# c0rv4x/zkevm-prover

Measured on AMD Instinct MI355X. Metric: batch-proof STARK sec (2^23 trace) + Goldilocks NTT Gelem/s at 1/2/4/8 GPU, lower is better.
Workload: dtype u64 (Goldilocks) + F_p^3

## Files before the change

### zkevm-prover_amd/csrc/ntt.hip

```cpp
#include <stdlib.h>
#include <string.h>

#include <algorithm>
#include <utility>
#include <vector>

#include "gl_device.hpp"
#include "gl_rb.hpp"
#include "zkgpu_internal.hpp"

namespace zk {

__global__ void k_fill_powers(uint64_t *out, uint64_t base, uint64_t step, uint64_t scale, uint64_t count)
{
    uint64_t i = (uint64_t)blockIdx.x * blockDim.x + threadIdx.x;
    if (i >= count) return;
    uint64_t b = gl_pow(base, step);
    out[i] = gl_canon(gl_mul(scale, gl_pow(b, i)));
}

__device__ __forceinline__ uint32_t bitrev_u32(uint32_t x, uint32_t bits)
{
    return bits == 0 ? 0 : (__builtin_bitreverse32(x) >> (32 - bits));
}

__device__ __forceinline__ uint64_t tw_big(const uint64_t *lo, const uint64_t *hi, uint64_t e)
{
    return gl_mul(lo[e & (TW_LEVEL_SIZE - 1)], hi[e >> TW_LEVEL_BITS]);
}

struct PassArgs {
    const uint64_t *src;
    uint64_t src_ld;
    uint64_t src_valid;
    uint32_t half_zero;
    uint64_t *dst;
    uint64_t dst_ld;
    const uint64_t *tw_lo;
    const uint64_t *tw_hi;
    const uint64_t *post_lo;
    const uint64_t *post_hi;
    uint64_t post_step;
    uint64_t post_scale;
    uint32_t post_bits;
    uint32_t logn;
    uint32_t logm;
    uint32_t last;
    uint32_t npass;
    uint32_t rbits[NTT_MAX_PASSES];
    const uint64_t *otw;
    const uint64_t *rt4096;
    uint32_t ncols;
};

constexpr int GROUPS = 16;

#ifndef ZKGPU_NTT_RB
#define ZKGPU_NTT_RB 1
#endif
#ifndef ZKGPU_NTT_RB_SHIFT
#define ZKGPU_NTT_RB_SHIFT 1
#endif
template <bool RB>
__device__ __forceinline__ uint64_t bf_add(uint64_t a, uint64_t b)
{
    if constexpr (RB && ZKGPU_NTT_RB) return gl_add_rb(a, b);
    else return gl_add(a, b);
}
template <bool RB>
__device__ __forceinline__ uint64_t bf_sub(uint64_t a, uint64_t b)
{
    if constexpr (RB && ZKGPU_NTT_RB) return gl_sub_rb(a, b);
    else return gl_sub(a, b);
}

template <int E, bool RB>
__device__ __forceinline__ uint64_t bf_mul2e(uint64_t x)
{
    if constexpr (RB && ZKGPU_NTT_RB && ZKGPU_NTT_RB_SHIFT) return mul2e_rb<E>(x);
    else return mul2e<E>(x);
}

template <bool INV, int H, int I, bool RB>
__device__ __forceinline__ uint64_t dif_odd(uint64_t a, uint64_t c)
{
    constexpr int e = (96 * I) / H;
    if constexpr (e == 0) return bf_sub<RB>(a, c);
    else if constexpr (!INV) return bf_mul2e<e, RB>(bf_sub<RB>(a, c));
    else return bf_mul2e<96 - e, RB>(bf_sub<RB>(c, a));
}

template <int LOG, bool INV, bool RB = false, int H = (1 << LOG) / 2>
__device__ __forceinline__ void dft_regs(uint64_t *v)
{
    if constexpr (H >= 1) {
        constexpr int R = 1 << LOG;
        [&]<int... Bs>(std::integer_sequence<int, Bs...>) {
            (
                [&]<int B>() {
                    [&]<int... Is>(std::integer_sequence<int, Is...>) {
                        (
                            [&]<int I>() {
                                uint64_t a = v[B * 2 * H + I];
                                uint64_t c = v[B * 2 * H + I + H];
                                v[B * 2 * H + I] = bf_add<RB>(a, c);
                                v[B * 2 * H + I + H] = dif_odd<INV, H, I, RB>(a, c);
                            }.template operator()<Is>(),
                            ...);
                    }(std::make_integer_sequence<int, H>{});
                }.template operator()<Bs>(),
                ...);
        }(std::make_integer_sequence<int, R / (2 * H)>{});
        dft_regs<LOG, INV, RB, H / 2>(v);
    }
}

template <int LOG, bool INV, bool RB = false>
__device__ __forceinline__ void dft_regs_half(uint64_t *v)
{
    constexpr int R = 1 << LOG, H = R / 2;
    [&]<int... Is>(std::integer_sequence<int, Is...>) {
        ([&]<int I>() {
            constexpr int e = (96 * I) / H;
            static_assert(!INV, "forward only");
            if constexpr (e == 0) v[I + H] = v[I];
            else v[I + H] = mul2e<e>(v[I]);
        }.template operator()<Is>(), ...);
    }(std::make_integer_sequence<int, H>{});
    dft_regs<LOG, INV, RB, H / 2>(v);
}

__host__ __device__ constexpr int brev_c(int x, int bits)
{
    int r = 0;
    for (int i = 0; i < bits; i++) r |= ((x >> i) & 1) << (bits - 1 - i);
    return r;
}

template <int L1, int L2, bool INV, bool SPLIT>
__global__ void __launch_bounds__(16 * (1 << L2)) k_ntt_pass(PassArgs a)
{
    constexpr int R1 = 1 << L1, R2 = 1 << L2, LOGR = L1 + L2, R = 1 << LOGR;
    constexpr int T = GROUPS * R2;
    __shared__ uint64_t lds[SPLIT ? R * 8 : R * 17];
    uint32_t *lds32 = reinterpret_cast<uint32_t *>(lds);

    __shared__ uint64_t twR[R];
    const uint32_t col = blockIdx.x % a.ncols;
    const uint64_t u = blockIdx.x / a.ncols;
    const uint64_t *src = a.src + (uint64_t)col * a.src_ld;
    uint64_t *dst = a.dst + (uint64_t)col * a.dst_ld;
    const int tid = threadIdx.x;

    static_assert(LOGR <= 12, "radix");
    if (a.rt4096)
        for (int i = tid; i < R; i += T) twR[i] = a.rt4096[i << (12 - LOGR)];
    else
        for (int i = tid; i < R; i += T) twR[i] = tw_big(a.tw_lo, a.tw_hi, (uint64_t)i << (TW_MAX_LOG - LOGR));

    uint64_t v[R2 > R1 ? R2 : R1];
    int g, j2;
    uint64_t base = 0, k1g = 0, rest = 0;
    uint32_t logmp = 0, logS = 0;
    if (!a.last) {
        g = tid & 15;
        j2 = tid >> 4;
        logmp = a.logm - LOGR;
        const uint64_t groups_per_blk = 1ULL << (logmp - 4);
        const uint64_t blk = u >> (logmp - 4);
        const uint64_t j0 = (u & (groups_per_blk - 1)) << 4;
        base = (blk << a.logm) + j0;
#pragma unroll
        for (int j1 = 0; j1 < R1; j1++) {
            uint64_t pos = base + ((uint64_t)(R2 * j1 + j2) << logmp) + g;
            v[j1] = pos < a.src_valid ? src[pos] : 0;
        }
    } else {
        j2 = tid & (R2 - 1);
        g = tid >> L2;
        logS = a.logn - a.rbits[0] - LOGR;
        rest = u & ((1ULL << logS) - 1);
        k1g = u >> logS;
        const uint64_t blk = ((k1g * 16 + g) << logS) + rest;
#pragma unroll
        for (int j1 = 0; j1 < R1; j1++) {
            uint64_t pos = (blk << LOGR) + R2 * j1 + j2;
            v[j1] = pos < a.src_valid ? src[pos] : 0;
        }
    }
    if constexpr (!INV) {
        if (a.half_zero)
            dft_regs_half<L1, INV, true>(v);
        else
            dft_regs<L1, INV, true>(v);
    } else {
        dft_regs<L1, INV, true>(v);
    }
    __syncthreads();
#pragma unroll
    for (int r = 0; r < R1; r++) {
        const int k1 = brev_c(r, L1);
        if (k1) v[r] = gl_mul_rb(v[r], twR[(j2 * k1) & (R - 1)]);
    }
    const bool active = tid < GROUPS * R1;
    const int g2 = tid & 15, k1s = tid >> 4;
    if constexpr (SPLIT) {
        uint32_t lo[R2 > R1 ? R2 : R1];
        const int wb0 = (j2 << 4) + g, wb1 = ((j2 ^ 1) << 4) + g;
        const int fm = (k1s & 1) << 4;
        const int rbe = k1s * R2 * 16 + g2 + fm, rbo = k1s * R2 * 16 + g2 - fm;
#pragma unroll
        for (int r = 0; r < R1; r++) {
            const int k1 = brev_c(r, L1);
            lds32[k1 * R2 * 16 + ((k1 & 1) ? wb1 : wb0)] = (uint32_t)v[r];
        }
        __syncthreads();
        if (active) {
#pragma unroll
            for (int jj = 0; jj < R2; jj++) lo[jj] = lds32[((jj & 1) ? rbo : rbe) + (jj << 4)];
        }
        __syncthreads();
#pragma unroll
        for (int r = 0; r < R1; r++) {
            const int k1 = brev_c(r, L1);
            lds32[k1 * R2 * 16 + ((k1 & 1) ? wb1 : wb0)] = (uint32_t)(v[r] >> 32);
        }
        __syncthreads();
        if (!active) return;
#pragma unroll
        for (int jj = 0; jj < R2; jj++) v[jj] = ((uint64_t)lds32[((jj & 1) ? rbo : rbe) + (jj << 4)] << 32) | lo[jj];
    } else {
#pragma unroll
        for (int r = 0; r < R1; r++) lds[(brev_c(r, L1) * R2 + j2) * 17 + g] = v[r];
        __syncthreads();
        if (!active) return;
#pragma unroll
        for (int jj = 0; jj < R2; jj++) v[jj] = lds[(k1s * R2 + jj) * 17 + g2];
    }
    g = g2;
    const int k1 = k1s;
    dft_regs<L2, INV, true>(v);
    if (!a.last && a.otw) {
        const uint64_t jp = (base & ((1ULL << logmp) - 1)) + g;
#pragma unroll
        for (int k2 = 0; k2 < R2; k2++) {
            const int r = brev_c(k2, L2);
            const uint64_t k = (uint64_t)(k1 + R1 * k2);
            uint64_t x = v[r];
            if (k1 | k2) x = gl_mul_rb(x, a.otw[(k << logmp) + jp]);
            dst[base + (k << logmp) + g] = x;
        }
    } else if (!a.last) {
        const uint32_t tshift = TW_MAX_LOG - a.logm;
        const uint64_t jp = (base & ((1ULL << logmp) - 1)) + g;
        uint64_t t = tw_big(a.tw_lo, a.tw_hi, (jp * k1) << tshift);
        const uint64_t step = tw_big(a.tw_lo, a.tw_hi, (jp * R1) << tshift);
#pragma unroll
        for (int k2 = 0; k2 < R2; k2++) {
            const int r = brev_c(k2, L2);
            uint64_t x = v[r];
            if (k1 | k2) x = gl_mul(x, t);
            dst[base + ((uint64_t)(k1 + R1 * k2) << logmp) + g] = x;
            t = gl_mul(t, step);
        }
    } else {
        uint64_t rrev = 0;
        {
            uint32_t rev_pos[NTT_MAX_PASSES];
            uint32_t acc = 0;
            for (uint32_t i = 1; i + 1 < a.npass; i++) {
                rev_pos[i] = acc;
                acc += a.rbits[i];
            }
            uint64_t rr = rest;
            for (int i = (int)a.npass - 2; i >= 1; i--) {
                uint64_t d = rr & ((1ULL << a.rbits[i]) - 1);
                rr >>= a.rbits[i];
                rrev |= d << rev_pos[i];
            }
        }
        const uint32_t lognr = a.logn - LOGR;
        const uint64_t x0 = (k1g * 16 + g) + (rrev << a.rbits[0]) + ((uint64_t)k1 << lognr);
        const bool scaled = a.post_lo != nullptr || a.post_scale != 1;
        uint64_t f = a.post_scale;
        if (a.post_lo) f = gl_mul(a.post_lo[x0 & ((1ULL << a.post_bits) - 1)], a.post_hi[x0 >> a.post_bits]);
#pragma unroll
        for (int k2 = 0; k2 < R2; k2++) {
            const int r = brev_c(k2, L2);
            uint64_t x = v[r];
            if (scaled) x = gl_mul(x, f);
            dst[x0 + ((uint64_t)(R1 * k2) << lognr)] = gl_canon(x);
            if (a.post_lo) f = gl_mul(f, a.post_step);
        }
    }
}

constexpr int PASS_THREADS = 256;

struct SmallArgs {
    const uint64_t *src;
    uint64_t src_ld;
    uint64_t src_valid;
    uint64_t *dst;
    uint64_t dst_ld;
    const uint64_t *rt_small;
    const uint64_t *post_lo;
    const uint64_t *post_hi;
    uint64_t post_scale;
    uint32_t post_bits;
    uint32_t logn;
};

__global__ void __launch_bounds__(PASS_THREADS) k_ntt_small(SmallArgs a)
{
    __shared__ uint64_t lds[4096];
    const uint32_t col = blockIdx.x;
    const uint64_t *src = a.src + (uint64_t)col * a.src_ld;
    uint64_t *dst = a.dst + (uint64_t)col * a.dst_ld;
    const uint32_t n = 1u << a.logn;
    for (uint32_t i = threadIdx.x; i < n; i += PASS_THREADS) lds[i] = i < a.src_valid ? src[i] : 0;
    for (int lh = (int)a.logn - 1; lh >= 0; lh--) {
        const uint32_t h = 1u << lh;
        __syncthreads();
        for (uint32_t b = threadIdx.x; b < n / 2; b += PASS_THREADS) {
            uint32_t pos = b & (h - 1);
            uint32_t i0 = ((b >> lh) << (lh + 1)) + pos;
            uint32_t i1 = i0 + h;
            uint64_t x = lds[i0], y = lds[i1];
            lds[i0] = gl_add(x, y);
            uint64_t d = gl_sub(x, y);
            lds[i1] = pos == 0 ? d : gl_mul(d, a.rt_small[pos << (11 - lh)]);
        }
    }
    __syncthreads();
    for (uint32_t k = threadIdx.x; k < n; k += PASS_THREADS) {
        uint64_t v = lds[bitrev_u32(k, a.logn)];
        if (a.post_lo)
            v = gl_mul(v, gl_mul(a.post_lo[k & ((1u << a.post_bits) - 1)], a.post_hi[k >> a.post_bits]));
        else if (a.post_scale != 1)
            v = gl_mul(v, a.post_scale);
        dst[k] = gl_canon(v);
    }
}

__global__ void k_rows_to_cols(const uint64_t *__restrict__ in, uint64_t *__restrict__ out, uint64_t nrows,
                               uint64_t ncols, uint64_t ld)
{
    __shared__ uint64_t tile[32][33];
    uint64_t r0 = (uint64_t)blockIdx.x * 32, c0 = (uint64_t)blockIdx.y * 32;
    int tx = threadIdx.x & 31, ty = threadIdx.x >> 5;
    for (int k = ty; k < 32; k += 8) {
        uint64_t r = r0 + k, c = c0 + tx;
        if (r < nrows && c < ncols) tile[k][tx] = in[r * ncols + c];
    }
    __syncthreads();
    for (int k = ty; k < 32; k += 8) {
        uint64_t c = c0 + k, r = r0 + tx;
        if (r < nrows && c < ncols) out[c * ld + r] = tile[tx][k];
    }
}

__global__ void k_cols_to_rows(const uint64_t *__restrict__ in, uint64_t *__restrict__ out, uint64_t nrows,
                               uint64_t ncols, uint64_t ld)
{
    __shared__ uint64_t tile[32][33];
    uint64_t r0 = (uint64_t)blockIdx.x * 32, c0 = (uint64_t)blockIdx.y * 32;
    int tx = threadIdx.x & 31, ty = threadIdx.x >> 5;
    for (int k = ty; k < 32; k += 8) {
        uint64_t c = c0 + k, r = r0 + tx;
        if (r < nrows && c < ncols) tile[k][tx] = in[c * ld + r];
    }
    __syncthreads();
    for (int k = ty; k < 32; k += 8) {
        uint64_t r = r0 + k, c = c0 + tx;
        if (r < nrows && c < ncols) out[r * ncols + c] = tile[tx][k];
    }
}

__global__ void k_otw_table(uint64_t *out, const uint64_t *tw_lo, const uint64_t *tw_hi, uint32_t logm,
                            uint32_t logr)
{
    const uint64_t i = (uint64_t)blockIdx.x * blockDim.x + threadIdx.x;
    if (i >> logm) return;
    const uint32_t logmp = logm - logr;
    const uint64_t k = i >> logmp, jp = i & ((1ULL << logmp) - 1);
    out[i] = gl_canon(tw_big(tw_lo, tw_hi, (jp * k) << (TW_MAX_LOG - logm)));
}

constexpr uint32_t OTW_MAX_LOG = 24;
struct OtwTable {
    int d;
    uint32_t logm, logr;
    uint64_t *ptr;
};
static std::vector<OtwTable> g_otw;

static const uint64_t *otw_table(Ctx &ctx, int d, uint32_t logm, uint32_t logr, hipStream_t s)
{
    if (logm > OTW_MAX_LOG) return nullptr;
    for (const OtwTable &t : g_otw)
        if (t.d == d && t.logm == logm && t.logr == logr) return t.ptr;
    uint64_t *p = nullptr;
    const uint64_t m = 1ULL << logm;
    if (hipMalloc((void **)&p, m * sizeof(uint64_t)) != hipSuccess) {
        (void)hipGetLastError();
        return nullptr;
    }
    hipLaunchKernelGGL(k_otw_table, dim3((uint32_t)((m + 255) / 256)), dim3(256), 0, s, p, ctx.tw_lo[d], ctx.tw_hi[d],
                       logm, logr);
    g_otw.push_back(OtwTable{d, logm, logr, p});
    return p;
}

static const char *PASS_NAMES[2][9] = {
    {"", "", "", "", "k_ntt_pass<4,fwd>", "k_ntt_pass<5,fwd>", "k_ntt_pass<6,fwd>", "k_ntt_pass<7,fwd>",
     "k_ntt_pass<8,fwd>"},
    {"", "", "", "", "k_ntt_pass<4,inv>", "k_ntt_pass<5,inv>", "k_ntt_pass<6,inv>", "k_ntt_pass<7,inv>",
     "k_ntt_pass<8,inv>"}};
static const char *PASS_NAMES_REC[2][9] = {
    {"", "", "", "", "k_ntt_pass<4,fwd,rec>", "k_ntt_pass<5,fwd,rec>", "k_ntt_pass<6,fwd,rec>",
     "k_ntt_pass<7,fwd,rec>", "k_ntt_pass<8,fwd,rec>"},
    {"", "", "", "", "k_ntt_pass<4,inv,rec>", "k_ntt_pass<5,inv,rec>", "k_ntt_pass<6,inv,rec>",
     "k_ntt_pass<7,inv,rec>", "k_ntt_pass<8,inv,rec>"}};

static bool otw_tables_enabled()
{
    const char *e = getenv("ZKGPU_NTT_OTW");
    return !(e && strcmp(e, "0") == 0);
}

static void split_radix(uint32_t logn, uint32_t *npass, uint32_t rbits[NTT_MAX_PASSES])
{
    uint32_t P = (logn + 7) / 8;
    *npass = P;
    uint32_t base = logn / P, extra = logn % P;
    for (uint32_t i = 0; i < P; i++) rbits[i] = base + (i >= P - extra ? 1 : 0);
}

template <int L1, int L2>
static void launch_pass(const PassArgs &a, uint64_t ncols, int inverse, hipStream_t s)
{
    constexpr int LOGR = L1 + L2;
    uint64_t units = (1ULL << (a.logn - LOGR)) / 16;
    dim3 grid((uint32_t)(units * ncols));
    if (inverse)
        hipLaunchKernelGGL((k_ntt_pass<L1, L2, true, true>), grid, dim3(16 << L2), 0, s, a);
    else
        hipLaunchKernelGGL((k_ntt_pass<L1, L2, false, true>), grid, dim3(16 << L2), 0, s, a);
}

static void dispatch_pass(uint32_t logr, const PassArgs &a, uint64_t ncols, int inverse, hipStream_t s)
{
    switch (logr) {
    case 4: launch_pass<2, 2>(a, ncols, inverse, s); break;
    case 5: launch_pass<2, 3>(a, ncols, inverse, s); break;
    case 6: launch_pass<3, 3>(a, ncols, inverse, s); break;
    case 7: launch_pass<3, 4>(a, ncols, inverse, s); break;
    case 8: launch_pass<4, 4>(a, ncols, inverse, s); break;
    default: break;
    }
}

int ntt_columns(Ctx &ctx, uint64_t *dst, uint64_t dst_ld, const uint64_t *src, uint64_t src_ld, uint64_t src_valid,
                uint64_t *tmp, uint64_t tmp_ld, uint32_t logn, uint64_t ncols, int inverse, const uint64_t *post_lo,
                const uint64_t *post_hi, uint32_t post_bits, uint64_t post_base, uint64_t post_scale, hipStream_t s)
{
    if (ncols == 0) return 0;
    if (logn > TW_MAX_LOG) return set_error(ZKGPU_ERR_ARG, "ntt: log2(n) exceeds %u", TW_MAX_LOG);
    const int d = inverse ? 1 : 0;
    if (logn <= 12) {
        SmallArgs sa;
        sa.src = src;
        sa.src_ld = src_ld;
        sa.src_valid = src_valid;
        sa.dst = dst;
        sa.dst_ld = dst_ld;
        sa.rt_small = ctx.rt_small[d];
        sa.post_lo = post_lo;
        sa.post_hi = post_hi;
        sa.post_bits = post_bits;
        sa.post_scale = post_scale;
        sa.logn = logn;
        for (uint64_t c0 = 0; c0 < ncols; c0 += 65535) {
            uint64_t nc = ncols - c0 < 65535 ? ncols - c0 : 65535;
            SmallArgs b = sa;
            b.src = src + c0 * src_ld;
            b.dst = dst + c0 * dst_ld;
            const uint64_t n = 1ULL << logn;
            const uint64_t nread = (src_valid < n ? src_valid : n);
            prof_begin(s);
            hipLaunchKernelGGL(k_ntt_small, dim3((uint32_t)nc), dim3(PASS_THREADS), 0, s, b);
            prof_end("k_ntt_small", 8.0 * (double)(nread + n) * (double)nc, s);
        }
        return check_launch("k_ntt_small");
    }
    PassArgs a;
    a.rt4096 = ctx.rt_small[d];
    a.tw_lo = ctx.tw_lo[d];
    a.tw_hi = ctx.tw_hi[d];
    a.logn = logn;
    split_radix(logn, &a.npass, a.rbits);
    const bool use_otw = otw_tables_enabled();
    uint32_t logm = logn;
    for (uint32_t p = 0; p < a.npass; p++) {
        a.logm = logm;
        a.last = (p == a.npass - 1);
        a.post_lo = a.last ? post_lo : nullptr;
        a.post_hi = a.last ? post_hi : nullptr;
        a.post_bits = post_bits;
        a.post_scale = a.last ? post_scale : 1;
        const uint32_t rb = a.rbits[p];
        a.post_step = h_pow(post_base, (uint64_t)(1u << (rb / 2)) << (logn - rb));
        a.otw = (a.last || !use_otw) ? nullptr : otw_table(ctx, d, logm, rb, s);
        const char *name = (!a.last && !a.otw) ? PASS_NAMES_REC[d][rb] : PASS_NAMES[d][rb];
        a.half_zero = 0;
        if (p == 0) {
            a.src = src;
            a.src_ld = src_ld;
            a.src_valid = src_valid;
            const uint32_t l1 = rb / 2;
            a.half_zero = (!inverse && l1 >= 1 && src_valid == (1ULL << (logn - 1))) ? 1u : 0u;
        } else {
            a.src = tmp;
            a.src_ld = tmp_ld;
            a.src_valid = ~0ULL;
        }
        if (a.last) {
            a.dst = dst;
            a.dst_ld = dst_ld;
        } else {
            a.dst = tmp;
            a.dst_ld = tmp_ld;
        }
        const uint64_t n = 1ULL << logn;
        const uint64_t nread = (a.src_valid < n ? a.src_valid : n);
        const uint64_t units = (1ULL << (logn - rb)) / 16;
        const uint64_t cmax = std::max<uint64_t>(1, std::min<uint64_t>(65535, (1ULL << 32) / (units * 256)));
        for (uint64_t c0 = 0; c0 < ncols; c0 += cmax) {
            uint64_t nc = ncols - c0 < cmax ? ncols - c0 : cmax;
            PassArgs b = a;
            b.src = a.src + c0 * a.src_ld;
            b.dst = a.dst + c0 * a.dst_ld;
            b.ncols = (uint32_t)nc;
            prof_begin(s);
            dispatch_pass(rb, b, nc, inverse, s);
            prof_end(name, 8.0 * (double)(nread + n) * (double)nc, s);
        }
        logm -= rb;
    }
    return check_launch("k_ntt_pass");
}

void rows_to_cols(const uint64_t *in, uint64_t *out, uint64_t nrows, uint64_t ncols, uint64_t ld, hipStream_t s)
{
    if (!nrows || !ncols) return;
    dim3 grid((uint32_t)((nrows + 31) / 32), (uint32_t)((ncols + 31) / 32));
    hipLaunchKernelGGL(k_rows_to_cols, grid, dim3(256), 0, s, in, out, nrows, ncols, ld);
}

void cols_to_rows(const uint64_t *in, uint64_t *out, uint64_t nrows, uint64_t ncols, uint64_t ld, hipStream_t s)
{
    if (!nrows || !ncols) return;
    dim3 grid((uint32_t)((nrows + 31) / 32), (uint32_t)((ncols + 31) / 32));
    hipLaunchKernelGGL(k_cols_to_rows, grid, dim3(256), 0, s, in, out, nrows, ncols, ld);
}

void fill_powers(uint64_t *out, uint64_t base, uint64_t step, uint64_t scale, uint64_t count, hipStream_t s)
{
    uint32_t blocks = (uint32_t)((count + 255) / 256);
    hipLaunchKernelGGL(k_fill_powers, dim3(blocks), dim3(256), 0, s, out, base, step, scale, count);
}


constexpr int LDE_LB = 12;
constexpr uint64_t LDE_RB = 1ULL << LDE_LB;
constexpr int SP_THREADS = 256;

struct StridedArgs {
    const uint64_t *src;
    uint64_t src_ld;
    uint64_t *dst;
    uint64_t dst_ld;
    uint64_t row_stride;
    const uint64_t *tw_r;
    const uint64_t *otw;
    uint32_t canon;
    uint32_t ncols;
    uint32_t units;
};

template <int LA, bool INV>
__global__ void __launch_bounds__(SP_THREADS) k_lde_strided(StridedArgs a)
{
    constexpr int LT = LA - 6, T = 1 << LT, G = SP_THREADS / T, M = 64 / T;
    constexpr int ROW = T * G + (G < 32 ? G : 0);
    __shared__ uint32_t lds[64 * ROW];
    const uint32_t col = blockIdx.x % a.ncols;
    const uint64_t unit = blockIdx.x / a.ncols;
    const uint64_t g0 = unit * G;
    const int tid = threadIdx.x, g = tid % G, t = tid / G;
    const uint64_t rs = a.row_stride;
    const uint64_t *src = a.src + (uint64_t)col * a.src_ld + g0 + g;
    uint64_t v[64];
#pragma unroll
    for (int j1 = 0; j1 < 64; j1++) v[j1] = src[(uint64_t)(t + T * j1) * rs];
    dft_regs<6, INV>(v);
    if constexpr (T > 1) {
#pragma unroll
        for (int r = 1; r < 64; r++) v[r] = gl_mul(v[r], a.tw_r[t * brev_c(r, 6)]);
    }
    const int wb = t * G + g;
#pragma unroll
    for (int r = 0; r < 64; r++) lds[brev_c(r, 6) * ROW + wb] = (uint32_t)v[r];
    __syncthreads();
    uint32_t nl[64];
#pragma unroll
    for (int m = 0; m < M; m++)
#pragma unroll
        for (int j2 = 0; j2 < T; j2++) nl[m * T + j2] = lds[(t + T * m) * ROW + j2 * G + g];
    __syncthreads();
#pragma unroll
    for (int r = 0; r < 64; r++) lds[brev_c(r, 6) * ROW + wb] = (uint32_t)(v[r] >> 32);
    __syncthreads();
#pragma unroll
    for (int m = 0; m < M; m++)
#pragma unroll
        for (int j2 = 0; j2 < T; j2++)
            v[m * T + j2] = ((uint64_t)lds[(t + T * m) * ROW + j2 * G + g] << 32) | nl[m * T + j2];
#pragma unroll
    for (int m = 0; m < M; m++) dft_regs<LT, INV>(v + m * T);
    uint64_t *dst = a.dst + (uint64_t)col * a.dst_ld + g0 + g;
    const uint64_t *otw = a.otw ? a.otw + g0 + g : nullptr;
#pragma unroll
    for (int m = 0; m < M; m++) {
#pragma unroll
        for (int r = 0; r < T; r++) {
            const uint64_t k = (uint64_t)(t + T * m) + 64 * (uint64_t)brev_c(r, LT);
            uint64_t x = v[m * T + r];
            if (otw) x = gl_mul(x, otw[k * LDE_RB]);
            dst[k * rs] = a.canon ? gl_canon(x) : x;
        }
    }
}

struct MidArgs {
    const uint64_t *src;
    uint64_t src_ld;
    uint64_t *dst;
    uint64_t dst_ld;
    const uint64_t *tw16[2];
    const uint64_t *tw256[2];
    const uint64_t *fs;
    const uint64_t *twa[2];
    const uint64_t *otw;
    uint64_t nblk;
    uint32_t ncols;
};

constexpr int MID_LDS = 16 * 272;

#ifndef ZKGPU_LDE_MID_RB
#define ZKGPU_LDE_MID_RB 0
#endif
__device__ __forceinline__ uint64_t mid_mul(uint64_t a, uint64_t b)
{
    if constexpr (ZKGPU_LDE_MID_RB) return gl_mul_rb(a, b);
    else return gl_mul(a, b);
}

template <bool INV, bool TA>
__device__ __forceinline__ void dft4096_block(uint64_t *v, uint64_t *L, int t, const uint64_t *tw16,
                                              const uint64_t *tw256)
{
    dft_regs<4, INV, ZKGPU_LDE_MID_RB>(v);
    if constexpr (TA) {
#pragma unroll
        for (int r = 0; r < 16; r++) v[r] = mid_mul(v[r], tw16[(brev_c(r, 4) << 8) + t]);
    } else {
#pragma unroll
        for (int r = 1; r < 16; r++) v[r] = mid_mul(v[r], tw16[t * brev_c(r, 4)]);
    }
#pragma unroll
    for (int r = 0; r < 16; r++) L[brev_c(r, 4) * 272 + t] = v[r];
    __syncthreads();
    __builtin_amdgcn_sched_barrier(0);
    const int lo = t & 15, hi = t >> 4;
#pragma unroll
    for (int j1 = 0; j1 < 16; j1++) v[j1] = L[hi * 272 + lo + 16 * j1];
    __syncthreads();
    __builtin_amdgcn_sched_barrier(0);
    dft_regs<4, INV, ZKGPU_LDE_MID_RB>(v);
#pragma unroll
    for (int r = 1; r < 16; r++) v[r] = mid_mul(v[r], tw256[lo * brev_c(r, 4)]);
#pragma unroll
    for (int r = 0; r < 16; r++) L[lo * 257 + brev_c(r, 4) * 16 + hi] = v[r];
    __syncthreads();
    __builtin_amdgcn_sched_barrier(0);
#pragma unroll
    for (int j0 = 0; j0 < 16; j0++) v[j0] = L[j0 * 257 + hi * 16 + lo];
    __syncthreads();
    __builtin_amdgcn_sched_barrier(0);
    dft_regs<4, INV, ZKGPU_LDE_MID_RB>(v);
}

__global__ void __launch_bounds__(256) __attribute__((amdgpu_waves_per_eu(2, 2))) k_lde_mid(MidArgs a)
{
    __shared__ uint64_t L[MID_LDS];
    const int t = threadIdx.x;
    const uint64_t blk = blockIdx.x;
    const uint32_t col = (uint32_t)(blk % a.ncols);
    const uint64_t kA = blk / a.ncols;
    const uint64_t *src = a.src + (uint64_t)col * a.src_ld + kA * LDE_RB + t;
    uint64_t v[16], c[16];
#pragma unroll
    for (int j = 0; j < 16; j++) v[j] = src[256 * j];
    dft4096_block<true, false>(v, L, t, a.tw16[1], a.tw256[1]);
    __builtin_amdgcn_sched_barrier(0);
#pragma unroll
    for (int k = 0; k < 16; k++) c[k] = v[brev_c(k, 4)];
    uint64_t *dst = a.dst + (uint64_t)col * a.dst_ld + kA * 2 * LDE_RB + 2 * t;
    const uint64_t *otw = a.otw + kA * LDE_RB + t;
    const uint64_t RA = a.nblk / a.ncols;
    uint64_t z0[16];
    for (int p = 0; p < 2; p++) {
        const uint64_t *S = a.fs + ((uint64_t)p * RA + kA) * 16;
#pragma unroll
        for (int k = 0; k < 16; k++) v[k] = mid_mul(c[k], S[k]);
        dft4096_block<false, true>(v, L, t, a.twa[p], a.tw256[0]);
        __builtin_amdgcn_sched_barrier(0);
        if (p == 0) {
#pragma unroll
            for (int k = 0; k < 16; k++) z0[k] = v[k];
        }
    }
#pragma unroll
    for (int k = 0; k < 16; k++) {
        const uint64_t w = otw[256 * k];
        HIP_vector_type<unsigned long long, 2> pr;
        pr.x = mid_mul(z0[brev_c(k, 4)], w);
        pr.y = mid_mul(v[brev_c(k, 4)], w);
        *reinterpret_cast<HIP_vector_type<unsigned long long, 2> *>(dst + 512 * k) = pr;
    }
}

struct Lde3Tables {
    uint32_t logn = 0;
    uint64_t *pow16[2] = {nullptr, nullptr}, *pow256[2] = {nullptr, nullptr}, *powR[2] = {nullptr, nullptr};
    uint64_t *fs = nullptr, *twa = nullptr;
};

__global__ void k_lde_fs(uint64_t *fs, uint64_t F, uint64_t ninv, uint64_t RA)
{
    const uint64_t i = (uint64_t)blockIdx.x * blockDim.x + threadIdx.x;
    if (i >= RA * 16) return;
    const uint64_t kA = i >> 4, k = i & 15;
    fs[i] = gl_canon(gl_mul(ninv, gl_pow(F, kA + 256 * RA * k)));
}

__global__ void k_lde_twa(uint64_t *twa, uint64_t F, uint64_t w4096, uint64_t RA)
{
    const uint32_t i = blockIdx.x * blockDim.x + threadIdx.x;
    if (i >= 4096) return;
    const uint64_t k2 = i >> 8, t = i & 255;
    twa[i] = gl_canon(gl_mul(gl_pow(F, RA * t), gl_pow(w4096, t * k2)));
}
static Lde3Tables g_lde3;

static int lde3_tables(Ctx &ctx, uint32_t logn, hipStream_t s)
{
    Lde3Tables &T = g_lde3;
    if (T.logn == logn) return 0;
    const uint32_t la = logn - LDE_LB;
    const uint64_t RA = 1ULL << la, n = 1ULL << logn;
    auto alloc = [&](uint64_t **p, uint64_t count) -> int {
        if (*p) (void)hipFree(*p);
        *p = nullptr;
        if (hipMalloc((void **)p, count * 8) != hipSuccess) return set_error(ZKGPU_ERR_OOM, "lde tables");
        return 0;
    };
    int rc;
    for (int d = 0; d < 2; d++) {
        const uint64_t w16 = d ? h_inv(h_w(12)) : h_w(12), w256 = d ? h_inv(h_w(8)) : h_w(8),
                       wR = d ? h_inv(h_w(la)) : h_w(la);
        if ((rc = alloc(&T.pow16[d], 4096)) || (rc = alloc(&T.pow256[d], 256)) || (rc = alloc(&T.powR[d], RA)))
            return rc;
        fill_powers(T.pow16[d], w16, 1, 1, 4096, s);
        fill_powers(T.pow256[d], w256, 1, 1, 256, s);
        fill_powers(T.powR[d], wR, 1, 1, RA, s);
    }
    if ((rc = alloc(&T.fs, 2 * RA * 16)) || (rc = alloc(&T.twa, 2 * 4096))) return rc;
    const uint64_t ninv = h_inv(n);
    for (int p = 0; p < 2; p++) {
        const uint64_t F = p ? h_mul(7, h_w(logn + 1)) : 7;
        hipLaunchKernelGGL(k_lde_fs, dim3((uint32_t)((RA * 16 + 255) / 256)), dim3(256), 0, s, T.fs + p * RA * 16, F,
                           ninv, RA);
        hipLaunchKernelGGL(k_lde_twa, dim3(16), dim3(256), 0, s, T.twa + p * 4096, F, h_w(12), RA);
    }
    if ((rc = check_launch("lde tables"))) return rc;
    T.logn = logn;
    return 0;
}

template <int LA>
static void launch_strided(const StridedArgs &a, uint64_t units, int inverse, hipStream_t s)
{
    const dim3 grid((uint32_t)(units * a.ncols));
    if (inverse) hipLaunchKernelGGL((k_lde_strided<LA, true>), grid, dim3(SP_THREADS), 0, s, a);
    else hipLaunchKernelGGL((k_lde_strided<LA, false>), grid, dim3(SP_THREADS), 0, s, a);
}

static void dispatch_strided(uint32_t la, StridedArgs a, uint64_t groups, int inverse, hipStream_t s)
{
    const uint64_t units = groups / (SP_THREADS >> (la - 6));
    a.units = (uint32_t)units;
    switch (la) {
    case 6: launch_strided<6>(a, units, inverse, s); break;
    case 7: launch_strided<7>(a, units, inverse, s); break;
    case 8: launch_strided<8>(a, units, inverse, s); break;
    case 9: launch_strided<9>(a, units, inverse, s); break;
    case 10: launch_strided<10>(a, units, inverse, s); break;
    case 11: launch_strided<11>(a, units, inverse, s); break;
    case 12: launch_strided<12>(a, units, inverse, s); break;
    default: break;
    }
}

bool lde3_supported(uint32_t logn, uint32_t loge)
{
    const char *e = getenv("ZKGPU_LDE3");
    const bool enabled = e && atoi(e) != 0;
    return enabled && loge == logn + 1 && logn >= LDE_LB + 6 && logn <= LDE_LB + 12;
}

static const char *P1_NAMES[13] = {"", "", "", "", "", "", "k_lde_p1<6>", "k_lde_p1<7>", "k_lde_p1<8>", "k_lde_p1<9>",
                                   "k_lde_p1<10>", "k_lde_p1<11>", "k_lde_p1<12>"};
static const char *P3_NAMES[13] = {"", "", "", "", "", "", "k_lde_p3<6>", "k_lde_p3<7>", "k_lde_p3<8>", "k_lde_p3<9>",
                                   "k_lde_p3<10>", "k_lde_p3<11>", "k_lde_p3<12>"};

int lde3_columns(Ctx &ctx, uint64_t *out, uint64_t ld_out, const uint64_t *in, uint64_t ld_in, uint64_t *t1,
                 uint32_t logn, uint64_t ncols, hipStream_t s)
{
    if (logn < LDE_LB + 6 || logn > LDE_LB + 12) return set_error(ZKGPU_ERR_ARG, "lde3: unsupported size 2^%u", logn);
    if (ncols == 0) return 0;
    int rc;
    if ((rc = lde3_tables(ctx, logn, s))) return rc;
    const uint32_t la = logn - LDE_LB;
    const uint64_t n = 1ULL << logn, RA = 1ULL << la;
    const uint64_t *otw_inv = otw_table(ctx, 1, logn, la, s), *otw_fwd = otw_table(ctx, 0, logn, la, s);
    if (!otw_inv || !otw_fwd) return set_error(ZKGPU_ERR_OOM, "lde3: twiddle tables");
    const uint64_t cmax = std::min<uint64_t>(65535, (1ULL << 31) / (2 * LDE_RB));
    for (uint64_t c0 = 0; c0 < ncols; c0 += cmax) {
        const uint32_t nc = (uint32_t)std::min<uint64_t>(cmax, ncols - c0);
        StridedArgs p1;
        p1.src = in + c0 * ld_in;
        p1.src_ld = ld_in;
        p1.dst = t1;
        p1.dst_ld = n;
        p1.row_stride = LDE_RB;
        p1.tw_r = g_lde3.powR[1];
        p1.otw = otw_inv;
        p1.canon = 0;
        p1.ncols = nc;
        prof_begin(s);
        dispatch_strided(la, p1, LDE_RB, 1, s);
        prof_end(P1_NAMES[la], 16.0 * (double)n * nc, s);
        MidArgs m;
        m.src = t1;
        m.src_ld = n;
        m.dst = out + c0 * ld_out;
        m.dst_ld = ld_out;
        for (int d = 0; d < 2; d++) {
            m.tw16[d] = g_lde3.pow16[d];
            m.tw256[d] = g_lde3.pow256[d];
            m.twa[d] = g_lde3.twa + d * 4096;
        }
        m.fs = g_lde3.fs;
        m.otw = otw_fwd;
        m.nblk = RA * nc;
        m.ncols = nc;
        prof_begin(s);
        hipLaunchKernelGGL(k_lde_mid, dim3((uint32_t)m.nblk), dim3(256), 0, s, m);
        prof_end("k_lde_mid", 24.0 * (double)n * nc, s);
        StridedArgs p3;
        p3.src = out + c0 * ld_out;
        p3.src_ld = ld_out;
        p3.dst = out + c0 * ld_out;
        p3.dst_ld = ld_out;
        p3.row_stride = 2 * LDE_RB;
        p3.tw_r = g_lde3.powR[0];
        p3.otw = nullptr;
        p3.canon = 1;
        p3.ncols = nc;
        prof_begin(s);
        dispatch_strided(la, p3, 2 * LDE_RB, 0, s);
        prof_end(P3_NAMES[la], 32.0 * (double)n * nc, s);
    }
    return check_launch("lde3");
}

}
```

Before: 0.2404.

## Specialize NTT pass kernel by role, input and post mode with scalar-base addressing

Splits the NTT pass kernel into compile-time variants for twiddle-table, recomputed-twiddle and last passes, for full, half-zero and bounds-checked inputs, and for each post-scaling mode, removing runtime branches. Loads and stores use a scalar base pointer plus a 32-bit byte offset, and block indices are forced uniform, so address arithmetic is cheaper and VGPR pressure is lower. In table mode the output twiddles are prefetched a few iterations ahead to hide load latency. The twiddle setup now always reads rt4096, which assumes that table is always present, and 32-bit offsets cap the addressable size.

New measurement: 0.2344, median of 6. 2.5% less time.

```diff
diff --git a/zkevm-prover_amd/csrc/ntt.hip b/zkevm-prover_amd/csrc/ntt.hip
--- a/zkevm-prover_amd/csrc/ntt.hip
+++ b/zkevm-prover_amd/csrc/ntt.hip
@@ -137,65 +137,82 @@
     return r;
 }
 
-template <int L1, int L2, bool INV, bool SPLIT>
+enum : int { ROLE_TAB = 0, ROLE_REC = 1, ROLE_LAST = 2 };
+enum : int { IN_FULL = 0, IN_HALF = 1, IN_CHECK = 2 };
+enum : int { POST_NONE = 0, POST_SCALE = 1, POST_TABLE = 2 };
+
+template <class T>
+__device__ __forceinline__ T *sgpr_ptr(T *p)
+{
+    asm("" : "+s"(p));
+    return p;
+}
+#define ZK_GLOBAL __attribute__((address_space(1)))
+__device__ __forceinline__ uint64_t ld_off(const uint64_t *base, uint32_t byte_off)
+{
+    return *(const ZK_GLOBAL uint64_t *)((const ZK_GLOBAL char *)sgpr_ptr(base) + byte_off);
+}
+__device__ __forceinline__ void st_off(uint64_t *base, uint32_t byte_off, uint64_t x)
+{
+    *(ZK_GLOBAL uint64_t *)((ZK_GLOBAL char *)sgpr_ptr(base) + byte_off) = x;
+}
+
+constexpr int NTT_OTW_AHEAD = 4;
+
+template <int L1, int L2, bool INV, bool SPLIT, int ROLE, int IN, int POST>
 __global__ void __launch_bounds__(16 * (1 << L2)) k_ntt_pass(PassArgs a)
 {
     constexpr int R1 = 1 << L1, R2 = 1 << L2, LOGR = L1 + L2, R = 1 << LOGR;
     constexpr int T = GROUPS * R2;
+    constexpr bool LAST = ROLE == ROLE_LAST;
+    static_assert(!(LAST && IN != IN_FULL) && !(!LAST && POST != POST_NONE) && !(INV && IN == IN_HALF), "role");
     __shared__ uint64_t lds[SPLIT ? R * 8 : R * 17];
     uint32_t *lds32 = reinterpret_cast<uint32_t *>(lds);
 
     __shared__ uint64_t twR[R];
-    const uint32_t col = blockIdx.x % a.ncols;
-    const uint64_t u = blockIdx.x / a.ncols;
+    const uint32_t col = __builtin_amdgcn_readfirstlane(blockIdx.x % a.ncols);
+    const uint32_t u = __builtin_amdgcn_readfirstlane(blockIdx.x / a.ncols);
     const uint64_t *src = a.src + (uint64_t)col * a.src_ld;
     uint64_t *dst = a.dst + (uint64_t)col * a.dst_ld;
     const int tid = threadIdx.x;
 
     static_assert(LOGR <= 12, "radix");
-    if (a.rt4096)
-        for (int i = tid; i < R; i += T) twR[i] = a.rt4096[i << (12 - LOGR)];
-    else
-        for (int i = tid; i < R; i += T) twR[i] = tw_big(a.tw_lo, a.tw_hi, (uint64_t)i << (TW_MAX_LOG - LOGR));
+    for (int i = tid; i < R; i += T) twR[i] = a.rt4096[i << (12 - LOGR)];
 
     uint64_t v[R2 > R1 ? R2 : R1];
     int g, j2;
-    uint64_t base = 0, k1g = 0, rest = 0;
-    uint32_t logmp = 0, logS = 0;
-    if (!a.last) {
+    uint64_t base = 0;
+    uint32_t j0 = 0, k1g = 0, rest = 0, logmp = 0, logS = 0;
+    if constexpr (!LAST) {
         g = tid & 15;
         j2 = tid >> 4;
         logmp = a.logm - LOGR;
-        const uint64_t groups_per_blk = 1ULL << (logmp - 4);
-        const uint64_t blk = u >> (logmp - 4);
-        const uint64_t j0 = (u & (groups_per_blk - 1)) << 4;
-        base = (blk << a.logm) + j0;
-#pragma unroll
-        for (int j1 = 0; j1 < R1; j1++) {
-            uint64_t pos = base + ((uint64_t)(R2 * j1 + j2) << logmp) + g;
-            v[j1] = pos < a.src_valid ? src[pos] : 0;
+        const uint32_t blk = u >> (logmp - 4);
+        j0 = (u & ((1u << (logmp - 4)) - 1)) << 4;
+        base = ((uint64_t)blk << a.logm) + j0;
+        const uint64_t rstride = (uint64_t)R2 << logmp;
+        const uint32_t off = ((uint32_t)j2 << logmp) + g;
+        const uint64_t *s = src + base;
+#pragma unroll
+        for (int j1 = 0; j1 < (IN == IN_HALF ? R1 / 2 : R1); j1++) {
+            if constexpr (IN == IN_CHECK)
+                v[j1] = base + j1 * rstride + off < a.src_valid ? ld_off(s + j1 * rstride, off * 8) : 0;
+            else
+                v[j1] = ld_off(s + j1 * rstride, off * 8);
         }
     } else {
         j2 = tid & (R2 - 1);
         g = tid >> L2;
         logS = a.logn - a.rbits[0] - LOGR;
-        rest = u & ((1ULL << logS) - 1);
+        rest = u & ((1u << logS) - 1);
         k1g = u >> logS;
-        const uint64_t blk = ((k1g * 16 + g) << logS) + rest;
-#pragma unroll
-        for (int j1 = 0; j1 < R1; j1++) {
-            uint64_t pos = (blk << LOGR) + R2 * j1 + j2;
-            v[j1] = pos < a.src_valid ? src[pos] : 0;
-        }
-    }
-    if constexpr (!INV) {
-        if (a.half_zero)
-            dft_regs_half<L1, INV, true>(v);
-        else
-            dft_regs<L1, INV, true>(v);
-    } else {
-        dft_regs<L1, INV, true>(v);
-    }
+        const uint64_t *s = src + (((((uint64_t)k1g * 16) << logS) + rest) << LOGR);
+        const uint32_t off = ((uint32_t)g << (logS + LOGR)) + j2;
+#pragma unroll
+        for (int j1 = 0; j1 < R1; j1++) v[j1] = ld_off(s + R2 * j1, off * 8);
+    }
+    if constexpr (IN == IN_HALF) dft_regs_half<L1, INV, true>(v);
+    else dft_regs<L1, INV, true>(v);
     __syncthreads();
 #pragma unroll
     for (int r = 0; r < R1; r++) {
@@ -239,32 +256,44 @@
     }
     g = g2;
     const int k1 = k1s;
+    constexpr int OTW_AHEAD = ROLE != ROLE_TAB ? 0 : NTT_OTW_AHEAD < R2 ? NTT_OTW_AHEAD : R2;
+    uint64_t w[R2];
+    const uint64_t kstride_t = (uint64_t)R1 << logmp;
+    const uint32_t off_t = (((uint32_t)k1 << logmp) + g) * 8;
+    const uint64_t *ot = a.otw + j0;
+    if constexpr (ROLE == ROLE_TAB) {
+#pragma unroll
+        for (int k2 = 0; k2 < OTW_AHEAD; k2++) w[k2] = ld_off(ot + k2 * kstride_t, off_t);
+    }
     dft_regs<L2, INV, true>(v);
-    if (!a.last && a.otw) {
-        const uint64_t jp = (base & ((1ULL << logmp) - 1)) + g;
+    if constexpr (ROLE == ROLE_TAB) {
+        uint64_t *d = dst + base;
 #pragma unroll
         for (int k2 = 0; k2 < R2; k2++) {
             const int r = brev_c(k2, L2);
-            const uint64_t k = (uint64_t)(k1 + R1 * k2);
             uint64_t x = v[r];
-            if (k1 | k2) x = gl_mul_rb(x, a.otw[(k << logmp) + jp]);
-            dst[base + (k << logmp) + g] = x;
-        }
-    } else if (!a.last) {
+            if (k1 | k2) x = gl_mul_rb(x, w[k2]);
+            if (k2 + OTW_AHEAD < R2) w[k2 + OTW_AHEAD] = ld_off(ot + (k2 + OTW_AHEAD) * kstride_t, off_t);
+            st_off(d + k2 * kstride_t, off_t, x);
+        }
+    } else if constexpr (ROLE == ROLE_REC) {
         const uint32_t tshift = TW_MAX_LOG - a.logm;
-        const uint64_t jp = (base & ((1ULL << logmp) - 1)) + g;
+        const uint64_t jp = (uint64_t)j0 + g;
         uint64_t t = tw_big(a.tw_lo, a.tw_hi, (jp * k1) << tshift);
         const uint64_t step = tw_big(a.tw_lo, a.tw_hi, (jp * R1) << tshift);
+        const uint64_t kstride = (uint64_t)R1 << logmp;
+        const uint32_t off = (((uint32_t)k1 << logmp) + g) * 8;
+        uint64_t *d = dst + base;
 #pragma unroll
         for (int k2 = 0; k2 < R2; k2++) {
             const int r = brev_c(k2, L2);
             uint64_t x = v[r];
             if (k1 | k2) x = gl_mul(x, t);
-            dst[base + ((uint64_t)(k1 + R1 * k2) << logmp) + g] = x;
+            st_off(d + k2 * kstride, off, x);
             t = gl_mul(t, step);
         }
     } else {
-        uint64_t rrev = 0;
+        uint32_t rrev = 0;
         {
             uint32_t rev_pos[NTT_MAX_PASSES];
             uint32_t acc = 0;
@@ -272,25 +301,30 @@
                 rev_pos[i] = acc;
                 acc += a.rbits[i];
             }
-            uint64_t rr = rest;
+            uint32_t rr = rest;
             for (int i = (int)a.npass - 2; i >= 1; i--) {
-                uint64_t d = rr & ((1ULL << a.rbits[i]) - 1);
+                uint32_t d = rr & ((1u << a.rbits[i]) - 1);
                 rr >>= a.rbits[i];
                 rrev |= d << rev_pos[i];
             }
         }
         const uint32_t lognr = a.logn - LOGR;
-        const uint64_t x0 = (k1g * 16 + g) + (rrev << a.rbits[0]) + ((uint64_t)k1 << lognr);
-        const bool scaled = a.post_lo != nullptr || a.post_scale != 1;
+        const uint32_t ub = k1g * 16 + (rrev << a.rbits[0]);
+        const uint32_t xoff = (uint32_t)g + ((uint32_t)k1 << lognr);
+        const uint64_t kstride = (uint64_t)R1 << lognr;
+        uint64_t *d = dst + ub;
         uint64_t f = a.post_scale;
-        if (a.post_lo) f = gl_mul(a.post_lo[x0 & ((1ULL << a.post_bits) - 1)], a.post_hi[x0 >> a.post_bits]);
+        if constexpr (POST == POST_TABLE) {
+            const uint32_t x0 = ub + xoff;
+            f = gl_mul(a.post_lo[x0 & (uint32_t)((1ULL << a.post_bits) - 1)], a.post_hi[x0 >> a.post_bits]);
+        }
 #pragma unroll
         for (int k2 = 0; k2 < R2; k2++) {
             const int r = brev_c(k2, L2);
             uint64_t x = v[r];
-            if (scaled) x = gl_mul(x, f);
-            dst[x0 + ((uint64_t)(R1 * k2) << lognr)] = gl_canon(x);
-            if (a.post_lo) f = gl_mul(f, a.post_step);
+            if constexpr (POST != POST_NONE) x = gl_mul(x, f);
+            st_off(d + k2 * kstride, xoff * 8, gl_canon(x));
+            if constexpr (POST == POST_TABLE) f = gl_mul(f, a.post_step);
         }
     }
 }
@@ -437,16 +471,46 @@
     for (uint32_t i = 0; i < P; i++) rbits[i] = base + (i >= P - extra ? 1 : 0);
 }
 
+template <int L1, int L2, bool INV, int ROLE, int IN, int POST>
+static void launch_inst(const PassArgs &a, dim3 grid, hipStream_t s)
+{
+    hipLaunchKernelGGL((k_ntt_pass<L1, L2, INV, true, ROLE, IN, POST>), grid, dim3(16 << L2), 0, s, a);
+}
+
+template <int L1, int L2, bool INV>
+static void launch_role(const PassArgs &a, dim3 grid, hipStream_t s)
+{
+    if (a.last) {
+        if (a.post_lo) launch_inst<L1, L2, INV, ROLE_LAST, IN_FULL, POST_TABLE>(a, grid, s);
+        else if (a.post_scale != 1) launch_inst<L1, L2, INV, ROLE_LAST, IN_FULL, POST_SCALE>(a, grid, s);
+        else launch_inst<L1, L2, INV, ROLE_LAST, IN_FULL, POST_NONE>(a, grid, s);
+        return;
+    }
+    const bool full = a.src_valid >= (1ULL << a.logn);
+    if constexpr (!INV) {
+        if (a.half_zero) {
+            if (a.otw) launch_inst<L1, L2, INV, ROLE_TAB, IN_HALF, POST_NONE>(a, grid, s);
+            else launch_inst<L1, L2, INV, ROLE_REC, IN_HALF, POST_NONE>(a, grid, s);
+            return;
+        }
+    }
+    if (full) {
+        if (a.otw) launch_inst<L1, L2, INV, ROLE_TAB, IN_FULL, POST_NONE>(a, grid, s);
+        else launch_inst<L1, L2, INV, ROLE_REC, IN_FULL, POST_NONE>(a, grid, s);
+    } else {
+        if (a.otw) launch_inst<L1, L2, INV, ROLE_TAB, IN_CHECK, POST_NONE>(a, grid, s);
+        else launch_inst<L1, L2, INV, ROLE_REC, IN_CHECK, POST_NONE>(a, grid, s);
+    }
+}
+
 template <int L1, int L2>
 static void launch_pass(const PassArgs &a, uint64_t ncols, int inverse, hipStream_t s)
 {
     constexpr int LOGR = L1 + L2;
     uint64_t units = (1ULL << (a.logn - LOGR)) / 16;
     dim3 grid((uint32_t)(units * ncols));
-    if (inverse)
-        hipLaunchKernelGGL((k_ntt_pass<L1, L2, true, true>), grid, dim3(16 << L2), 0, s, a);
-    else
-        hipLaunchKernelGGL((k_ntt_pass<L1, L2, false, true>), grid, dim3(16 << L2), 0, s, a);
+    if (inverse) launch_role<L1, L2, true>(a, grid, s);
+    else launch_role<L1, L2, false>(a, grid, s);
 }
 
 static void dispatch_pass(uint32_t logr, const PassArgs &a, uint64_t ncols, int inverse, hipStream_t s)
```
